# Aedelon/MASt3R-SLAM

Measured on AMD Instinct MI355X. Metric: keyframe-pairs/sec (512x512 two-view infer+match+GN), higher is better.
Workload: dtype fp16

## Files before the change

mast3r-slam_amd/csrc/conv_tail.hip:

```cpp
#include "gemm_common.h"

using namespace m3gemm;

namespace {

constexpr int kThreads = 512;
constexpr int TH = 16, TW = 32;
constexpr int HH = TH + 2, HW = TW + 2;
constexpr int kHaloPix = HH * HW;
constexpr int kHaloBytes = kHaloPix * 128;
constexpr int kWStage = 128 * 128;
constexpr int PH = 11, PW = 19;
constexpr int kPatchBytes = (PH * PW * 128 + 1023) / 1024 * 1024;
constexpr int kLdsBytes = kHaloBytes + 2 * kWStage + kPatchBytes;

struct TailArgs {
    const bf16_t *X;
    const bf16_t *Wc;
    const float *bias;
    const bf16_t *W4;
    const float *b4;
    float *pts, *conf;
    bf16_t *Y;
    const bf16_t *R;
    int cout, relu_in;
    const bf16_t *zero16;
    int B, H, W, IH, IW;
    const bf16_t *Wc2, *W42;
    const float *bias2, *b42;
    int wt;
};

enum { EP_PLAIN = 0 , EP_TAIL = 1 , EP_RELU = 2 ,
       EP_ADD = 3  };

template <int DT, bool UPS, int CIN, int EP>
__global__ void __launch_bounds__(kThreads, 2)
k_conv_tail(const TailArgs ain) {
    constexpr bool TAIL = EP == EP_TAIL;
    static_assert(CIN % 64 == 0 && (TAIL ? CIN == 128 : true), "64-channel steps; the fused tail is the 128-channel head.2");
    constexpr int NQ = CIN / 64;
    TailArgs a = ain;
    if (blockIdx.y == 1) {
        a.Wc = ain.Wc2; a.W4 = ain.W42; a.bias = ain.bias2; a.b4 = ain.b42;
        a.X = ain.X + (size_t)ain.B * ain.IH * ain.IW * CIN;
        if (TAIL) {
            a.pts = ain.pts + (size_t)ain.B * ain.H * ain.W * 3;
            a.conf = ain.conf + (size_t)ain.B * ain.H * ain.W;
        } else {
            a.Y = ain.Y + (size_t)ain.B * ain.H * ain.W * ain.cout;
            if (EP == EP_ADD) a.R = ain.R + (size_t)ain.B * ain.H * ain.W * ain.cout;
        }
    }
    if (!TAIL) {
        const int z = blockIdx.z;
        a.Wc += (size_t)z * 128 * 9 * CIN;
        if (a.bias) a.bias += z * 128;
        a.Y += z * 128;
        if (EP == EP_ADD) a.R += z * 128;
    }
    const auto y_rsrc = stream_rsrc(a.Y);
    extern __shared__ __attribute__((aligned(16))) unsigned char lds[];
    unsigned char *halo = lds, *wst = lds + kHaloBytes, *patch = lds + kHaloBytes + 2 * kWStage;
    const int tid = threadIdx.x, lane = tid & 63, wave = tid >> 6;
    const int wp = wave >> 1, wc = wave & 1;
    const int tiles_x = (a.W + TW - 1) / TW, tiles_y = a.H / TH;
    const int nwg = tiles_x * tiles_y * a.B;
    const int bid = xcd_remap(blockIdx.x, nwg);
    const int b = bid / (tiles_x * tiles_y), trem = bid - b * tiles_x * tiles_y;
    const int ty = trem / tiles_x, tx = trem - ty * tiles_x;
    const int oy0 = ty * TH, ox0 = tx * TW;
    const bf16_t *img = a.X + (size_t)b * a.IH * a.IW * CIN;

    const auto w_rsrc = stream_rsrc(a.Wc);
    const int wave_u = __builtin_amdgcn_readfirstlane(wave);
    unsigned char *const lds_wave = lds + wave_u * 1024;
    unsigned w_lane[2];
#pragma unroll
    for (int i = 0; i < 2; ++i) {
        const int slot = i * kThreads + tid;
        const int row = slot >> 3, cp = slot & 7;
        w_lane[i] = (unsigned)row * (9 * CIN * 2) + ((cp ^ ((row >> 1) & 7)) << 4);
    }
    auto stage_w = [&](int tap, int half, int buf) {
#pragma unroll
        for (int i = 0; i < 2; ++i)
            blds16(w_rsrc, w_lane[i], (unsigned)(tap * CIN + half * 64) * 2u,
                   lds_wave + kHaloBytes + buf * kWStage + i * (kThreads * 16));
    };
    const float sy = UPS && a.H > 1 ? (float)(a.IH - 1) / (float)(a.H - 1) : 0.f;
    const float sx = UPS && a.W > 1 ? (float)(a.IW - 1) / (float)(a.W - 1) : 0.f;
    const int py0 = (int)((float)max(oy0 - 1, 0) * sy), px0 = (int)((float)max(ox0 - 1, 0) * sx);
    constexpr int kPatchIss = (PH * PW * 8 + 63) / 64, kPatchPerWave = (kPatchIss + 7) / 8;
    const auto x_rsrc = stream_rsrc(img);
    unsigned p_lane[UPS ? kPatchPerWave : 1];
    if (UPS) {
#pragma unroll
        for (int j = 0; j < kPatchPerWave; ++j) {
            int slot = (wave + 8 * j) * 64 + lane;
            slot = slot < PH * PW * 8 ? slot : PH * PW * 8 - 1;
            const int pp = slot >> 3, c = slot & 7;
            const int y = min(py0 + pp / PW, a.IH - 1), x = min(px0 + pp % PW, a.IW - 1);
            p_lane[j] = (unsigned)((y * a.IW + x) * CIN + c * 8) * 2u;
        }
    }
    auto stage_patch = [&](int half) {
#pragma unroll
        for (int j = 0; j < kPatchPerWave; ++j)
            if (wave_u + 8 * j < kPatchIss)
                blds16(x_rsrc, p_lane[j], (unsigned)half * 128u, lds_wave + kHaloBytes + 2 * kWStage + j * 8192);
    };
    auto stage_halo_direct = [&](int half) {
        for (int wi = wave; wi < (kHaloPix * 8 + 63) / 64; wi += kThreads / 64) {
            int slot = wi * 64 + lane;
            const bool live = slot < kHaloPix * 8;
            slot = live ? slot : kHaloPix * 8 - 1;
            const int pix = slot >> 3, cp = slot & 7;
            const int hy = pix / HW, hx = pix - hy * HW;
            const int iy = oy0 + hy - 1, ix = ox0 + hx - 1;
            const int c = half * 8 + (cp ^ ((hx >> 1) & 7));
            const bool in = iy >= 0 && iy < a.H && ix >= 0 && ix < a.W;
            const void *src = in ? (const void *)(img + ((size_t)iy * a.IW + ix) * CIN + c * 8) : (const void *)a.zero16;
            if (wi * 64 + 64 <= kHaloPix * 8) glds16(src, halo + wi * 1024);
            else if (live) *reinterpret_cast<uint4 *>(halo + (size_t)slot * 16) = *reinterpret_cast<const uint4 *>(src);
        }
    };
    auto blend_halo = [&]() {
        for (int slot = tid; slot < kHaloPix * 8; slot += kThreads) {
            const int pix = slot >> 3, cp = slot & 7;
            const int hy = pix / HW, hx = pix - hy * HW;
            const int iy = oy0 + hy - 1, ix = ox0 + hx - 1;
            const int c = cp ^ ((hx >> 1) & 7);
            uint4 o = make_uint4(0u, 0u, 0u, 0u);
            if (iy >= 0 && iy < a.H && ix >= 0 && ix < a.W) {
                const float fy = iy * sy, fx = ix * sx;
                int y0 = (int)fy, x0 = (int)fx;
                y0 = min(y0, a.IH - 1); x0 = min(x0, a.IW - 1);
                const int y1 = min(y0 + 1, a.IH - 1), x1 = min(x0 + 1, a.IW - 1);
                const float wy = fy - (float)y0, wx = fx - (float)x0;
                const unsigned char *p = patch + c * 16;
                union U { uint4 q; unsigned w[4]; } q00, q01, q10, q11, r;
                q00.q = *reinterpret_cast<const uint4 *>(p + ((y0 - py0) * PW + (x0 - px0)) * 128);
                q01.q = *reinterpret_cast<const uint4 *>(p + ((y0 - py0) * PW + (x1 - px0)) * 128);
                q10.q = *reinterpret_cast<const uint4 *>(p + ((y1 - py0) * PW + (x0 - px0)) * 128);
                q11.q = *reinterpret_cast<const uint4 *>(p + ((y1 - py0) * PW + (x1 - px0)) * 128);
#pragma unroll
                for (int k = 0; k < 4; ++k) {
                    const float tl = lo16<DT>(q00.w[k]) * (1.f - wx) + lo16<DT>(q01.w[k]) * wx;
                    const float bl = lo16<DT>(q10.w[k]) * (1.f - wx) + lo16<DT>(q11.w[k]) * wx;
                    const float th = hi16<DT>(q00.w[k]) * (1.f - wx) + hi16<DT>(q01.w[k]) * wx;
                    const float bh = hi16<DT>(q10.w[k]) * (1.f - wx) + hi16<DT>(q11.w[k]) * wx;
                    r.w[k] = pack16<DT>(tl * (1.f - wy) + bl * wy, th * (1.f - wy) + bh * wy);
                }
                o = r.q;
            }
            *reinterpret_cast<uint4 *>(halo + (size_t)slot * 16) = o;
        }
    };

    f32x4 acc[8][4];
#pragma unroll
    for (int i = 0; i < 8; ++i)
#pragma unroll
        for (int j = 0; j < 4; ++j) acc[i][j] = f32x4{0.f, 0.f, 0.f, 0.f};
    const int frow = lane & 15, fch = lane >> 4;
    int w_off[4];
#pragma unroll
    for (int j = 0; j < 4; ++j) {
        const int r = wc * 64 + j * 16 + frow;
        w_off[j] = r * 128 + ((fch ^ ((r >> 1) & 7)) << 4);
    }

    const int group = wave >> 2;
    bf16x8 af[8], wf[4];
    const int pix_of_row = (int)((0x3D9F2A40E6C851B7ULL >> (4 * frow)) & 15);
    auto col_offset = [&](int hx) { return hx * 128 + ((fch ^ ((hx >> 1) & 7)) << 4); };
    auto read_frags = [&](int g, int tap, int ks) {
        const int ky = tap / 3, kx = tap - ky * 3;
        const unsigned char *wsrc = wst + (g & 1) * kWStage;
        const int flip = ks << 6;
        const int c0 = col_offset(pix_of_row + kx) ^ flip;
        const int c1 = col_offset(16 + pix_of_row + kx) ^ flip;
        const unsigned char *rowp = halo + (wp * 4 + ky) * (HW * 128);
#pragma unroll
        for (int j = 0; j < 4; ++j) wf[j] = *reinterpret_cast<const bf16x8 *>(wsrc + (w_off[j] ^ flip));
#pragma unroll
        for (int i = 0; i < 8; ++i)
            af[i] = *reinterpret_cast<const bf16x8 *>(rowp + (i >> 1) * (HW * 128) + ((i & 1) ? c1 : c0));
        if (!TAIL && a.relu_in) {
#pragma unroll
            for (int i = 0; i < 8; ++i) af[i] = relu_frag(af[i]);
        }
    };
    auto mfma_all = [&]() {
        __builtin_amdgcn_s_setprio(1);
#pragma unroll
        for (int i = 0; i < 8; ++i)
#pragma unroll
            for (int j = 0; j < 4; ++j) acc[i][j] = mfma16<DT>(wf[j], af[i], acc[i][j]);
        __builtin_amdgcn_s_setprio(0);
    };
    auto phase_end = [&]() {
        __builtin_amdgcn_sched_barrier(0);
        __builtin_amdgcn_s_barrier();
        __builtin_amdgcn_sched_barrier(0);
    };
    auto phase_end_wait = [&]() {
        __builtin_amdgcn_sched_barrier(0);
        asm volatile("s_waitcnt vmcnt(0)" ::: "memory");
        __builtin_amdgcn_s_barrier();
        __builtin_amdgcn_sched_barrier(0);
    };
    auto prefetch_w = [&](int g) { if (g + 1 < 9 * NQ) stage_w((g + 1) % 9, (g + 1) / 9, (g + 1) & 1); };
    auto run_half = [&](int half) {
        if (group == 0) {
#pragma unroll 1
            for (int tap = 0; tap < 9; ++tap) {
                const int g = half * 9 + tap;
                read_frags(g, tap, 0);
                prefetch_w(g);
                asm volatile("s_waitcnt lgkmcnt(0)" ::: "memory");
                phase_end();
                mfma_all();
                phase_end();
                read_frags(g, tap, 1);
                asm volatile("s_waitcnt lgkmcnt(0)" ::: "memory");
                phase_end();
                mfma_all();
                phase_end_wait();
            }
            phase_end();
        } else {
#pragma unroll 1
            for (int tap = 0; tap < 9; ++tap) {
                const int g = half * 9 + tap;
                if (tap > 0) mfma_all();
                phase_end();
                read_frags(g, tap, 0);
                prefetch_w(g);
                asm volatile("s_waitcnt lgkmcnt(0)" ::: "memory");
                phase_end();
                mfma_all();
                phase_end();
                read_frags(g, tap, 1);
                asm volatile("s_waitcnt lgkmcnt(0)" ::: "memory");
                phase_end_wait();
            }
            mfma_all();
            phase_end();
        }
    };

    stage_w(0, 0, 0);
    if (UPS) stage_patch(0); else stage_halo_direct(0);
    asm volatile("s_waitcnt vmcnt(0)" ::: "memory");
    lds_barrier();
#pragma unroll 1
    for (int q = 0; q < NQ; ++q) {
        if (UPS) {
            blend_halo();
            lds_barrier();
            if (q + 1 < NQ) stage_patch(q + 1);
        } else if (q > 0) {
            stage_halo_direct(q);
            asm volatile("s_waitcnt vmcnt(0)" ::: "memory");
            lds_barrier();
        }
        run_half(q);
    }

    if constexpr (EP == EP_ADD) {
        const int r = lane & 15, gq = lane >> 4;
        constexpr int RS = 272;
        unsigned char *wl = halo + wave * (32 * RS);
        float4 bj[4];
#pragma unroll
        for (int j = 0; j < 4; ++j)
            bj[j] = a.bias ? *reinterpret_cast<const float4 *>(a.bias + wc * 64 + j * 16 + gq * 4) : make_float4(0.f, 0.f, 0.f, 0.f);
        auto pix = [&](int pass, int rl, int &oy, int &ox) {
            const int i = pass * 2 + (rl >> 4);
            oy = oy0 + wp * 4 + (i >> 1);
            ox = ox0 + (i & 1) * 16 + (int)((0x3D9F2A40E6C851B7ULL >> (4 * (rl & 15))) & 15);
        };
        uint4 q[2][4];
        auto load_resid = [&](int pass, uint4 (&dst)[4]) {
#pragma unroll
            for (int it = 0; it < 4; ++it) {
                const int c = it * 64 + lane, rl = c >> 3, ch = c & 7;
                int oy, ox;
                pix(pass, rl, oy, ox);
                ox = ox < a.W ? ox : a.W - 1;
                dst[it] = *reinterpret_cast<const uint4 *>(a.R + (((size_t)b * a.H + oy) * a.W + ox) * a.cout + wc * 64 + ch * 8);
            }
        };
        load_resid(0, q[0]);
#pragma unroll
        for (int pass = 0; pass < 4; ++pass) {
            if (pass + 1 < 4) load_resid(pass + 1, q[(pass + 1) & 1]);
#pragma unroll
            for (int ii = 0; ii < 2; ++ii)
#pragma unroll
                for (int j = 0; j < 4; ++j) {
                    const f32x4 v = acc[pass * 2 + ii][j];
                    *reinterpret_cast<float4 *>(wl + (ii * 16 + r) * RS + ((j * 4 + gq) << 4)) =
                        make_float4(v[0] + bj[j].x, v[1] + bj[j].y, v[2] + bj[j].z, v[3] + bj[j].w);
                }
            asm volatile("s_waitcnt lgkmcnt(0)" ::: "memory");
#pragma unroll
            for (int it = 0; it < 4; ++it) {
                const int c = it * 64 + lane, rl = c >> 3, ch = c & 7;
                const float4 f0 = *reinterpret_cast<const float4 *>(wl + rl * RS + ch * 32);
                const float4 f1 = *reinterpret_cast<const float4 *>(wl + rl * RS + ch * 32 + 16);
                const uint4 u = q[pass & 1][it];
                uint4 o;
                o.x = pack16<DT>(f0.x + lo16<DT>(u.x), f0.y + hi16<DT>(u.x));
                o.y = pack16<DT>(f0.z + lo16<DT>(u.y), f0.w + hi16<DT>(u.y));
                o.z = pack16<DT>(f1.x + lo16<DT>(u.z), f1.y + hi16<DT>(u.z));
                o.w = pack16<DT>(f1.z + lo16<DT>(u.w), f1.w + hi16<DT>(u.w));
                int oy, ox;
                pix(pass, rl, oy, ox);
                if (ox < a.W)
                    store16_out<2>(a.wt != 0, y_rsrc, a.Y, (unsigned)((b * a.H + oy) * a.W + ox) * (unsigned)a.cout + wc * 64 + ch * 8,
                                   (((size_t)b * a.H + oy) * a.W + ox) * a.cout + wc * 64 + ch * 8, o);
            }
            asm volatile("" ::: "memory");
        }
    } else if constexpr (!TAIL) {
        const int r = lane & 15, gq = lane >> 4;
        unsigned char *wl = halo + wave * 8192;
        float4 bj[4];
#pragma unroll
        for (int j = 0; j < 4; ++j)
            bj[j] = a.bias ? *reinterpret_cast<const float4 *>(a.bias + wc * 64 + j * 16 + gq * 4) : make_float4(0.f, 0.f, 0.f, 0.f);
#pragma unroll
        for (int pass = 0; pass < 2; ++pass) {
#pragma unroll
            for (int ii = 0; ii < 4; ++ii)
#pragma unroll
                for (int j = 0; j < 4; ++j) {
                    f32x4 v = acc[pass * 4 + ii][j];
                    v[0] += bj[j].x; v[1] += bj[j].y; v[2] += bj[j].z; v[3] += bj[j].w;
                    if (EP == EP_RELU) {
#pragma unroll
                        for (int e = 0; e < 4; ++e) v[e] = v[e] > 0.f ? v[e] : 0.f;
                    }
                    uint2 pk;
                    pk.x = pack16<DT>(v[0], v[1]); pk.y = pack16<DT>(v[2], v[3]);
                    *reinterpret_cast<uint2 *>(wl + (ii * 16 + r) * 128 + (((j * 2 + (gq >> 1)) ^ ((r >> 1) & 7)) << 4) + (((gq ^ r) & 1) << 3)) = pk;
                }
            asm volatile("s_waitcnt lgkmcnt(0)" ::: "memory");
#pragma unroll
            for (int it = 0; it < 8; ++it) {
                const int c = it * 64 + lane, rl = c >> 3, ch = c & 7;
                uint4 v = *reinterpret_cast<const uint4 *>(wl + rl * 128 + ((ch ^ ((rl >> 1) & 7)) << 4));
                if (rl & 1) v = uint4{v.z, v.w, v.x, v.y};
                const int i = pass * 4 + (rl >> 4);
                const int oy = oy0 + wp * 4 + (i >> 1);
                const int ox = ox0 + (i & 1) * 16 + (int)((0x3D9F2A40E6C851B7ULL >> (4 * (rl & 15))) & 15);
                if (ox < a.W)
                    store16_out<2>(a.wt != 0, y_rsrc, a.Y, (unsigned)((b * a.H + oy) * a.W + ox) * (unsigned)a.cout + wc * 64 + ch * 8,
                                   (((size_t)b * a.H + oy) * a.W + ox) * a.cout + wc * 64 + ch * 8, v);
            }
            asm volatile("" ::: "memory");
        }
    } else {
        const int r = lane & 15, gq = lane >> 4;
        float part[8][4];
    #pragma unroll
        for (int i = 0; i < 8; ++i)
    #pragma unroll
            for (int o = 0; o < 4; ++o) part[i][o] = 0.f;
    #pragma unroll
        for (int j = 0; j < 4; ++j) {
            const int n = wc * 64 + j * 16 + gq * 4;
            const float4 bq = a.bias ? *reinterpret_cast<const float4 *>(a.bias + n) : make_float4(0.f, 0.f, 0.f, 0.f);
            float w4[4][4];
    #pragma unroll
            for (int o = 0; o < 4; ++o) {
                const uint2 q = *reinterpret_cast<const uint2 *>(a.W4 + (size_t)o * 128 + n);
                w4[o][0] = lo16<DT>(q.x); w4[o][1] = hi16<DT>(q.x); w4[o][2] = lo16<DT>(q.y); w4[o][3] = hi16<DT>(q.y);
            }
    #pragma unroll
            for (int i = 0; i < 8; ++i) {
                const f32x4 v = acc[i][j];
                const float h[4] = {fmaxf(v[0] + bq.x, 0.f), fmaxf(v[1] + bq.y, 0.f), fmaxf(v[2] + bq.z, 0.f), fmaxf(v[3] + bq.w, 0.f)};
    #pragma unroll
                for (int o = 0; o < 4; ++o)
                    part[i][o] += (h[0] * w4[o][0] + h[1] * w4[o][1]) + (h[2] * w4[o][2] + h[3] * w4[o][3]);
            }
        }
    #pragma unroll
        for (int i = 0; i < 8; ++i)
    #pragma unroll
            for (int o = 0; o < 4; ++o) {
                float v = part[i][o];
                v += __shfl_xor(v, 16, 64);
                v += __shfl_xor(v, 32, 64);
                part[i][o] = v;
            }
        float *red = reinterpret_cast<float *>(wst);
        if (gq == 0) {
    #pragma unroll
            for (int i = 0; i < 8; ++i)
                *reinterpret_cast<float4 *>(red + (((wp * 2 + wc) * 8 + i) * 16 + r) * 4) = make_float4(part[i][0], part[i][1], part[i][2], part[i][3]);
        }
        __syncthreads();
        {
            const int i = 4 * wc + gq;
            const float4 p0 = *reinterpret_cast<const float4 *>(red + (((wp * 2 + 0) * 8 + i) * 16 + r) * 4);
            const float4 p1 = *reinterpret_cast<const float4 *>(red + (((wp * 2 + 1) * 8 + i) * 16 + r) * 4);
            const int oy = oy0 + wp * 4 + (i >> 1), ox = ox0 + (i & 1) * 16 + pix_of_row;
            if (ox < a.W) {
                const float x = p0.x + p1.x + a.b4[0], y = p0.y + p1.y + a.b4[1];
                const float z = p0.z + p1.z + a.b4[2], c = p0.w + p1.w + a.b4[3];
                const float d = sqrtf(x * x + y * y + z * z);
                const float sc = expm1f(d) / fmaxf(d, 1e-8f);
                const size_t m = ((size_t)b * a.H + oy) * a.W + ox;
                a.pts[3 * m + 0] = x * sc; a.pts[3 * m + 1] = y * sc; a.pts[3 * m + 2] = z * sc;
                a.conf[m] = 1.0f + expf(c);
            }
        }
    }
}

}

extern "C" {

static int dpt_tail_launch(const void *X, const void *Wc, const float *bias, const void *W4, const float *b4,
                           const void *Wc2, const float *bias2, const void *W42, const float *b42, float *pts,
                           float *conf, void *Y, const void *R, const void *zero16, int B, int H, int W, int cin, int cout,
                           int ep, int relu_in, int upsample, int dtype, void *stream) {
    const int groups = Wc2 ? 2 : 1;
    const bool tail = ep == EP_TAIL;
    M3_REQUIRE(X && Wc && zero16 && B > 0 && H > 0 && W > 0 && H % 16 == 0 && W % 16 == 0);
    M3_REQUIRE(tail ? (W4 && b4 && pts && conf && cin == 128 && !Y)
                    : (Y && (cin == 128 || cin == 256) && (cout == 128 || cout == 256) && (ep == EP_PLAIN || ep == EP_RELU || ep == EP_ADD)));
    M3_REQUIRE((ep == EP_ADD) == (R != nullptr) && (!upsample || ep == EP_PLAIN || tail));
    M3_REQUIRE(groups == 1 || ((!tail || (W42 && b42)) && (bias == nullptr) == (bias2 == nullptr)));
    M3_REQUIRE((dtype == DT_BF16 || dtype == DT_F16) && (!upsample || (H % 2 == 0 && W % 2 == 0)));
    M3_REQUIRE((int64_t)groups * B * H * W < (1ll << 31));
    M3_REQUIRE(!upsample || (int64_t)(H / 2) * (W / 2) * cin * 2 < (1ll << 31) - 16);
    M3_REQUIRE(reinterpret_cast<uintptr_t>(X) % 16 == 0 && reinterpret_cast<uintptr_t>(Wc) % 16 == 0 &&
               reinterpret_cast<uintptr_t>(Y) % 16 == 0 && reinterpret_cast<uintptr_t>(R) % 16 == 0);
    TailArgs a;
    a.Wc2 = (const bf16_t *)Wc2; a.W42 = (const bf16_t *)W42; a.bias2 = bias2; a.b42 = b42;
    a.X = (const bf16_t *)X; a.Wc = (const bf16_t *)Wc; a.bias = bias; a.W4 = (const bf16_t *)W4; a.b4 = b4;
    a.pts = pts; a.conf = conf; a.Y = (bf16_t *)Y; a.R = (const bf16_t *)R; a.cout = tail ? 128 : cout; a.relu_in = relu_in;
    a.zero16 = (const bf16_t *)zero16; a.B = B; a.H = H; a.W = W;
    a.IH = upsample ? H / 2 : H; a.IW = upsample ? W / 2 : W;
    a.wt = !tail && out_fits32((long long)groups * B * H * W * cout, 2) ? 1 : 0;
    const dim3 grid((unsigned)((H / TH) * ((W + TW - 1) / TW) * B), groups, tail ? 1 : cout / 128), blk(kThreads);
    hipStream_t st = (hipStream_t)stream;
#define M3_TAIL(DTV, UP, CI, EPV)                                                                                \
    do {                                                                                                         \
        static M3AttrOnce once;                                                                                  \
        int dev__;                                                                                               \
        if (m3_attr_need(once, &dev__)) {                                                                        \
            M3_CHECK_HIP(hipFuncSetAttribute(reinterpret_cast<const void *>(&k_conv_tail<DTV, UP, CI, EPV>),     \
                                             hipFuncAttributeMaxDynamicSharedMemorySize, kLdsBytes), "m3_dpt_tail/attr"); \
            m3_attr_done(once, dev__);                                                                           \
        }                                                                                                        \
        hipLaunchKernelGGL((k_conv_tail<DTV, UP, CI, EPV>), grid, blk, kLdsBytes, st, a);                        \
    } while (0)
#define M3_TAIL_DT(UP, CI, EPV) do { if (dtype == DT_F16) M3_TAIL(DT_F16, UP, CI, EPV); else M3_TAIL(DT_BF16, UP, CI, EPV); } while (0)
    if (tail) { if (upsample) M3_TAIL_DT(true, 128, EP_TAIL); else M3_TAIL_DT(false, 128, EP_TAIL); }
    else if (ep == EP_PLAIN && cin == 128) { if (upsample) M3_TAIL_DT(true, 128, EP_PLAIN); else M3_TAIL_DT(false, 128, EP_PLAIN); }
    else if (ep == EP_PLAIN) { if (upsample) M3_TAIL_DT(true, 256, EP_PLAIN); else M3_TAIL_DT(false, 256, EP_PLAIN); }
    else if (ep == EP_RELU) { if (cin == 128) M3_TAIL_DT(false, 128, EP_RELU); else M3_TAIL_DT(false, 256, EP_RELU); }
    else { if (cin == 128) M3_TAIL_DT(false, 128, EP_ADD); else M3_TAIL_DT(false, 256, EP_ADD); }
#undef M3_TAIL_DT
#undef M3_TAIL
    M3_CHECK_LAUNCH("m3_dpt_tail");
    return M3_OK;
}

int m3_dpt_tail_grouped2_dt(const void *X, const void *Wc0, const void *Wc1, const float *bias0, const float *bias1,
                            const void *W40, const void *W41, const float *b40, const float *b41, float *pts,
                            float *conf, const void *zero16, int B, int H, int W, int upsample, int dtype, void *stream) {
    M3_REQUIRE(pts && conf && (Wc1 == nullptr) == (W41 == nullptr));
    if (!Wc1) bias1 = b41 = nullptr;
    return dpt_tail_launch(X, Wc0, bias0, W40, b40, Wc1, bias1, W41, b41, pts, conf, nullptr, nullptr, zero16, B, H, W, 128, 128,
                           EP_TAIL, 0, upsample, dtype, stream);
}

int m3_conv3x3_up_direct_grouped2_dt(const void *X, const void *Wc0, const void *Wc1, const float *bias0, const float *bias1,
                                     void *Y, const void *zero16, int B, int H, int W, int Cin, int upsample, int dtype,
                                     void *stream) {
    M3_REQUIRE(Y != nullptr);
    return dpt_tail_launch(X, Wc0, bias0, nullptr, nullptr, Wc1, Wc1 ? bias1 : nullptr, nullptr, nullptr, nullptr, nullptr, Y,
                           nullptr, zero16, B, H, W, Cin, 128, EP_PLAIN, 0, upsample, dtype, stream);
}

int m3_conv3x3_direct_grouped2_dt(const void *X, const void *W0, const void *W1, const float *bias0, const float *bias1,
                                  void *Y, const void *R, const void *zero16, int B, int H, int W, int Cin, int Cout,
                                  int epilogue, int dtype, void *stream) {
    const int relu_in = (epilogue & 0x100) ? 1 : 0;
    const int e = epilogue & 0xff;
    M3_REQUIRE(Y != nullptr && (e == M3_EPI_BF16 || e == M3_EPI_BF16_RELU || e == M3_EPI_BF16_ADD));
    const int ep = e == M3_EPI_BF16 ? EP_PLAIN : (e == M3_EPI_BF16_RELU ? EP_RELU : EP_ADD);
    return dpt_tail_launch(X, W0, bias0, nullptr, nullptr, W1, bias1, nullptr, nullptr, nullptr, nullptr, Y, R, zero16, B, H, W,
                           Cin, Cout, ep, relu_in, 0, dtype, stream);
}

}
```

Measured before the change: 302.1.

## Restructure bilinear upsample halo blend into separable row-streaming with reuse

Rewrites the halo bilinear-upsample blend so each lane owns a fixed column and streams down half the halo rows. Horizontally blended rows are carried over when the source row repeats, so adjacent output rows reuse them instead of reloading four corners per pixel. The two extra halo columns get their own small path, and a compile-time ablation macro can replace the blend with a plain copy. This cuts LDS loads and ALU work in the blend, but changes FMA ordering, which may shift rounding, and adds register pressure and loop-carried dependencies.

After: 304.8 (median of 6 runs). About the same (+0.9%).

```diff
diff --git a/mast3r-slam_amd/csrc/conv_tail.hip b/mast3r-slam_amd/csrc/conv_tail.hip
--- a/mast3r-slam_amd/csrc/conv_tail.hip
+++ b/mast3r-slam_amd/csrc/conv_tail.hip
@@ -1,6 +1,10 @@
 #include "gemm_common.h"
 
 using namespace m3gemm;
+
+#ifndef M3_CONV_ABL
+#define M3_CONV_ABL 0
+#endif
 
 namespace {
 
@@ -31,6 +35,37 @@
     int wt;
 };
 
+template <int DT>
+__device__ __forceinline__ void hblend8(const uint4 l, const uint4 r, float wx, float omwx, float (&t)[8]) {
+#pragma clang fp contract(off)
+    const unsigned lw[4] = {l.x, l.y, l.z, l.w}, rw[4] = {r.x, r.y, r.z, r.w};
+#pragma unroll
+    for (int k = 0; k < 4; ++k) {
+        const float rl = wx * lo16<DT>(rw[k]), lh = omwx * hi16<DT>(lw[k]);
+        t[2 * k] = __builtin_fmaf(omwx, lo16<DT>(lw[k]), rl);
+        t[2 * k + 1] = __builtin_fmaf(wx, hi16<DT>(rw[k]), lh);
+    }
+}
+template <int DT>
+__device__ __forceinline__ uint4 vblend8(const float (&top)[8], const float (&bot)[8], float wy, float omwy) {
+#pragma clang fp contract(off)
+    unsigned o[4];
+#pragma unroll
+    for (int k = 0; k < 4; ++k) {
+        const float tl = top[2 * k] * omwy, bh = bot[2 * k + 1] * wy;
+        o[k] = pack16<DT>(__builtin_fmaf(bot[2 * k], wy, tl), __builtin_fmaf(top[2 * k + 1], omwy, bh));
+    }
+    return make_uint4(o[0], o[1], o[2], o[3]);
+}
+__device__ __forceinline__ void blend_coord(int i, float s, int n, int &i0, int &i1, float &w, float &omw) {
+#pragma clang fp contract(off)
+    const float fi = (float)i;
+    i0 = min((int)(fi * s), n - 1);
+    i1 = min(i0 + 1, n - 1);
+    w = __builtin_fmaf(s, fi, -(float)i0);
+    omw = 1.f - w;
+}
+
 enum { EP_PLAIN = 0 , EP_TAIL = 1 , EP_RELU = 2 ,
        EP_ADD = 3  };
 
@@ -126,35 +161,83 @@
         }
     };
     auto blend_halo = [&]() {
-        for (int slot = tid; slot < kHaloPix * 8; slot += kThreads) {
-            const int pix = slot >> 3, cp = slot & 7;
-            const int hy = pix / HW, hx = pix - hy * HW;
-            const int iy = oy0 + hy - 1, ix = ox0 + hx - 1;
-            const int c = cp ^ ((hx >> 1) & 7);
-            uint4 o = make_uint4(0u, 0u, 0u, 0u);
-            if (iy >= 0 && iy < a.H && ix >= 0 && ix < a.W) {
-                const float fy = iy * sy, fx = ix * sx;
-                int y0 = (int)fy, x0 = (int)fx;
-                y0 = min(y0, a.IH - 1); x0 = min(x0, a.IW - 1);
-                const int y1 = min(y0 + 1, a.IH - 1), x1 = min(x0 + 1, a.IW - 1);
-                const float wy = fy - (float)y0, wx = fx - (float)x0;
-                const unsigned char *p = patch + c * 16;
-                union U { uint4 q; unsigned w[4]; } q00, q01, q10, q11, r;
-                q00.q = *reinterpret_cast<const uint4 *>(p + ((y0 - py0) * PW + (x0 - px0)) * 128);
-                q01.q = *reinterpret_cast<const uint4 *>(p + ((y0 - py0) * PW + (x1 - px0)) * 128);
-                q10.q = *reinterpret_cast<const uint4 *>(p + ((y1 - py0) * PW + (x0 - px0)) * 128);
-                q11.q = *reinterpret_cast<const uint4 *>(p + ((y1 - py0) * PW + (x1 - px0)) * 128);
-#pragma unroll
-                for (int k = 0; k < 4; ++k) {
-                    const float tl = lo16<DT>(q00.w[k]) * (1.f - wx) + lo16<DT>(q01.w[k]) * wx;
-                    const float bl = lo16<DT>(q10.w[k]) * (1.f - wx) + lo16<DT>(q11.w[k]) * wx;
-                    const float th = hi16<DT>(q00.w[k]) * (1.f - wx) + hi16<DT>(q01.w[k]) * wx;
-                    const float bh = hi16<DT>(q10.w[k]) * (1.f - wx) + hi16<DT>(q11.w[k]) * wx;
-                    r.w[k] = pack16<DT>(tl * (1.f - wy) + bl * wy, th * (1.f - wy) + bh * wy);
-                }
-                o = r.q;
-            }
-            *reinterpret_cast<uint4 *>(halo + (size_t)slot * 16) = o;
+        if (M3_CONV_ABL & 1) {
+            for (int slot = tid; slot < kHaloPix * 8; slot += kThreads)
+                *reinterpret_cast<uint4 *>(halo + (size_t)slot * 16) =
+                    *reinterpret_cast<const uint4 *>(patch + (size_t)min(slot, PH * PW * 8 - 1) * 16);
+            return;
+        }
+        struct Col { unsigned l, r, h; float w, omw; bool in; };
+        auto column = [&](int hx, int cp) {
+            const int ix = ox0 + hx - 1;
+            int x0, x1;
+            Col c;
+            blend_coord(min(max(ix, 0), a.W - 1), sx, a.IW, x0, x1, c.w, c.omw);
+            const unsigned ch = (unsigned)(cp ^ ((hx >> 1) & 7)) * 16u;
+            c.l = (unsigned)min(max(x0 - px0, 0), PW - 1) * 128u + ch;
+            c.r = (unsigned)min(max(x1 - px0, 0), PW - 1) * 128u + ch;
+            c.h = (unsigned)hx * 128u + (unsigned)cp * 16u;
+            c.in = ix >= 0 && ix < a.W;
+            return c;
+        };
+        struct Row { int p0, p1; float w, omw; bool in; };
+        auto row = [&](int hy) {
+            const int iy = oy0 + hy - 1;
+            int y0, y1;
+            Row r;
+            blend_coord(min(max(iy, 0), a.H - 1), sy, a.IH, y0, y1, r.w, r.omw);
+            r.p0 = min(max(y0 - py0, 0), PH - 1); r.p1 = min(max(y1 - py0, 0), PH - 1);
+            r.in = iy >= 0 && iy < a.H;
+            return r;
+        };
+        auto load_row = [&](int p, const Col &c, uint4 &l, uint4 &r) {
+            const unsigned char *src = patch + p * (PW * 128);
+            l = *reinterpret_cast<const uint4 *>(src + c.l);
+            r = *reinterpret_cast<const uint4 *>(src + c.r);
+        };
+        int ln = lane, td = tid;
+        asm volatile("" : "+v"(ln), "+v"(td));
+        if (td < 2 * HH * 8) {
+            const int hy = td >> 4;
+            const Col c = column(TW + ((td >> 3) & 1), td & 7);
+            const Row r = row(hy);
+            uint4 tl, tr, bl, br;
+            load_row(r.p0, c, tl, tr);
+            load_row(r.p1, c, bl, br);
+            float top[8], bot[8];
+            hblend8<DT>(tl, tr, c.w, c.omw, top);
+            hblend8<DT>(bl, br, c.w, c.omw, bot);
+            const uint4 o = vblend8<DT>(top, bot, r.w, r.omw);
+            *reinterpret_cast<uint4 *>(halo + hy * (HW * 128) + c.h) = c.in && r.in ? o : make_uint4(0u, 0u, 0u, 0u);
+        }
+        const Col c = column((wave_u & 3) * 8 + (ln >> 3), ln & 7);
+        const int hy0 = (wave_u >> 2) * (HH / 2);
+        unsigned char *dst = halo + hy0 * (HW * 128) + c.h;
+        Row r = row(hy0);
+        int p0 = __builtin_amdgcn_readfirstlane(r.p0);
+        float top[8], bot[8];
+        uint4 nl, nr;
+        {
+            uint4 tl, tr;
+            load_row(p0, c, tl, tr);
+            load_row(__builtin_amdgcn_readfirstlane(r.p1), c, nl, nr);
+            hblend8<DT>(tl, tr, c.w, c.omw, top);
+            hblend8<DT>(nl, nr, c.w, c.omw, bot);
+        }
+#pragma unroll 1
+        for (int j = 0; j < HH / 2; ++j) {
+            const Row rn = row(hy0 + min(j + 1, HH / 2 - 1));
+            const int pn = __builtin_amdgcn_readfirstlane(rn.p0);
+            const bool adv = pn != p0;
+            if (adv) load_row(__builtin_amdgcn_readfirstlane(rn.p1), c, nl, nr);
+            const uint4 o = vblend8<DT>(top, bot, r.w, r.omw);
+            *reinterpret_cast<uint4 *>(dst + j * (HW * 128)) = c.in && r.in ? o : make_uint4(0u, 0u, 0u, 0u);
+            if (adv) {
+#pragma unroll
+                for (int k = 0; k < 8; ++k) top[k] = bot[k];
+                hblend8<DT>(nl, nr, c.w, c.omw, bot);
+            }
+            r = rn; p0 = pn;
         }
     };
 
```
